# Qualcomm-AI-research/fastforward

Hardware: AMD Instinct MI355X
Metric: tokens/sec Llama-3-8B W8A8 quantized fwd; quant/dequant GB/s vs HBM peak (higher is better)
Workload: dtype int8; 1 GPU; llama3-8b shapes, W8 per-channel symmetric + A8 per-tensor asymmetric on the 7 linears x 32 layers (BASELINE.json configs[2] forward), weights re-quantized every step as in the reference; global_batch=8, seq_len=2048, parallelism=dp1 (batch-sharded replicas, no data-path collective), quantizers=448, launch=hipGraph replay

## Files before the change

fastforward_amd/csrc/ffq_common.h:

```cpp
#pragma once

#include <hip/hip_runtime.h>
#include <stdarg.h>
#include <stdint.h>
#include <stdio.h>

#include "../../include/ffq.h"

#ifndef FFQ_TICKET_ORDER
#define FFQ_TICKET_ORDER __ATOMIC_RELAXED
#endif
#define ffq_ticket_acquire()                                                      \
  do {                                                                            \
    if (FFQ_TICKET_ORDER != __ATOMIC_RELAXED) __builtin_amdgcn_fence(__ATOMIC_ACQUIRE, "agent"); \
  } while (0)

namespace ffq {

char* err_buf();
int fail(int code, const char* fmt, ...);
bool generic_kernels_forced();
bool mid_register_form_forced();
bool splitk_abandon_forced();
int check_launch(const char* what);

__host__ __device__ inline bool dt_valid(int dt) { return dt >= FFQ_F32 && dt <= FFQ_U8; }
__host__ __device__ inline bool dt_is_float(int dt) {
  return dt == FFQ_F32 || dt == FFQ_BF16 || dt == FFQ_F16 || dt == FFQ_F64;
}
__host__ __device__ inline int dt_size(int dt) {
  switch (dt) {
    case FFQ_F32: case FFQ_I32: return 4;
    case FFQ_BF16: case FFQ_F16: case FFQ_I16: return 2;
    case FFQ_F64: case FFQ_I64: return 8;
    default: return 1;
  }
}

__host__ __device__ inline float bf16_bits_to_f32(uint16_t h) {
  return __builtin_bit_cast(float, (uint32_t)h << 16);
}
__host__ __device__ inline uint16_t f32_to_bf16_bits(float f) {
  uint32_t u = __builtin_bit_cast(uint32_t, f);
  if (f != f) return 0x7FC0;
  u += 0x7FFFu + ((u >> 16) & 1u);
  return (uint16_t)(u >> 16);
}
__host__ __device__ inline float f16_bits_to_f32(uint16_t h) {
  return (float)__builtin_bit_cast(_Float16, h);
}
__host__ __device__ inline uint16_t f32_to_f16_bits(float f) {
  return __builtin_bit_cast(uint16_t, (_Float16)f);
}

__host__ __device__ inline float round_stage(float v, int dt) {
  if (dt == FFQ_BF16) return bf16_bits_to_f32(f32_to_bf16_bits(v));
  if (dt == FFQ_F16) return f16_bits_to_f32(f32_to_f16_bits(v));
  return v;
}

__host__ __device__ inline float rne(float v) { return __builtin_rintf(v); }
__host__ __device__ inline double rne(double v) { return __builtin_rint(v); }

__host__ __device__ inline float clamp_nan(float v, float lo, float hi) {
  float c = v < lo ? lo : v;
  c = c > hi ? hi : c;
  return v != v ? v : c;
}
__host__ __device__ inline double clamp_nan(double v, double lo, double hi) {
  double c = v < lo ? lo : v;
  c = c > hi ? hi : c;
  return v != v ? v : c;
}

__device__ inline double load_any(const void* p, int dt, int64_t i) {
  switch (dt) {
    case FFQ_F32: return (double)((const float*)p)[i];
    case FFQ_BF16: return (double)bf16_bits_to_f32(((const uint16_t*)p)[i]);
    case FFQ_F16: return (double)f16_bits_to_f32(((const uint16_t*)p)[i]);
    case FFQ_F64: return ((const double*)p)[i];
    case FFQ_I8: return (double)((const int8_t*)p)[i];
    case FFQ_I16: return (double)((const int16_t*)p)[i];
    case FFQ_I32: return (double)((const int32_t*)p)[i];
    case FFQ_I64: return (double)((const int64_t*)p)[i];
    default: return (double)((const uint8_t*)p)[i];
  }
}
__device__ inline void store_any(void* p, int dt, int64_t i, double v) {
  const bool nan = v != v;
  switch (dt) {
    case FFQ_F32: ((float*)p)[i] = (float)v; break;
    case FFQ_BF16: ((uint16_t*)p)[i] = f32_to_bf16_bits((float)v); break;
    case FFQ_F16: ((uint16_t*)p)[i] = f32_to_f16_bits((float)v); break;
    case FFQ_F64: ((double*)p)[i] = v; break;
    case FFQ_I8: ((int8_t*)p)[i] = nan ? 0 : (int8_t)(int64_t)v; break;
    case FFQ_I16: ((int16_t*)p)[i] = nan ? 0 : (int16_t)(int64_t)v; break;
    case FFQ_I32: ((int32_t*)p)[i] = nan ? INT32_MIN : (int32_t)(int64_t)v; break;
    case FFQ_I64: ((int64_t*)p)[i] = nan ? INT64_MIN : (int64_t)v; break;
    default: ((uint8_t*)p)[i] = nan ? 0 : (uint8_t)(int64_t)v; break;
  }
}

struct FastDiv {
  uint32_t mul;
  uint32_t shift;
  uint32_t div;
// ... 103 lines not shown
```

fastforward_amd/csrc/ffq_core.hip:

```cpp
#include "ffq_common.h"

#include <math.h>
#include <string.h>

namespace ffq {

static thread_local char g_err[512];

char* err_buf() { return g_err; }

int fail(int code, const char* fmt, ...) {
  va_list ap;
  va_start(ap, fmt);
  vsnprintf(g_err, sizeof g_err, fmt, ap);
  va_end(ap);
  return code;
}

int check_launch(const char* what) {
  hipError_t e = hipGetLastError();
  if (e != hipSuccess) return fail(FFQ_ERR_LAUNCH, "%s: %s", what, hipGetErrorString(e));
  return FFQ_OK;
}

// ... 85 lines not shown
                what, (long long)numel);
  return fail(FFQ_ERR_PARAM_NUMEL,
              "The size of tensor a (%lld) must match the size of tensor b (%lld) at non-singleton "
              "dimension 0 (%s vs number of tiles)",
              (long long)ntiles, (long long)numel, what);
}

GenericTiling make_generic(const ffq_tiling* t) {
  GenericTiling g;
  memset(&g, 0, sizeof g);
  g.ndim = t->ndim;
  int64_t s = 1;
  for (int k = t->ndim - 1; k >= 0; --k) {
    g.shape[k] = t->shape[k];
    g.tile[k] = t->tile[k];
    g.gstride[k] = s;
    s *= t->shape[k] / t->tile[k];
  }
  return g;
}

}

using namespace ffq;

extern "C" {

int ffq_abi_version(void) { return FFQ_ABI_VERSION; }
const char* ffq_last_error(void) { return err_buf(); }
const char* ffq_backend_name(void) { return "hip:gfx950"; }

int64_t ffq_num_tiles(const ffq_tiling* tiling) {
  TileInfo info;
  int rc = analyse(tiling, &info);
  if (rc) return -rc;
  return info.ntiles;
}

int ffq_promote_types(int a, int b) {
  if (!dt_valid(a) || !dt_valid(b)) return -FFQ_ERR_ARG;
  if (a == b) return a;
  const bool fa = dt_is_float(a), fb = dt_is_float(b);
  if (fa && !fb) return a;
  if (fb && !fa) return b;
  if (fa && fb) {
    if (a == FFQ_F64 || b == FFQ_F64) return FFQ_F64;
    return FFQ_F32;
  }
  if (a == FFQ_I64 || b == FFQ_I64) return FFQ_I64;
  if (a == FFQ_I32 || b == FFQ_I32) return FFQ_I32;
  return FFQ_I16;
}

int ffq_can_support_bitwidth(int dtype, double num_bits) {
  double avail;
  switch (dtype) {
    case FFQ_BF16: avail = 7; break;
    case FFQ_F16: avail = 10; break;
    case FFQ_F32: avail = 23; break;
    case FFQ_F64: avail = 52; break;
    case FFQ_I8: case FFQ_U8: avail = 8; break;
    case FFQ_I16: avail = 16; break;
    case FFQ_I32: avail = 32; break;
    case FFQ_I64: avail = 64; break;
    default: return 0;
  }
  return (avail + 2) >= num_bits;
}

int ffq_dequantize_result_dtype(int data_dt, int scale_dt, int offset_dt, int has_offset) {
  const int off_dt = has_offset ? offset_dt : scale_dt;
  const int add_dt = ffq_promote_types(data_dt, off_dt);
  if (add_dt < 0) return add_dt;
  return ffq_promote_types(add_dt, scale_dt);
}

}

namespace ffq {
static int g_force_generic = 0;
bool generic_kernels_forced() { return (__atomic_load_n(&g_force_generic, __ATOMIC_RELAXED) & 1) != 0; }
bool splitk_abandon_forced() { return (__atomic_load_n(&g_force_generic, __ATOMIC_RELAXED) & 2) != 0; }
bool mid_register_form_forced() { return (__atomic_load_n(&g_force_generic, __ATOMIC_RELAXED) & 4) != 0; }
}

extern "C" int ffq_force_generic_kernels(int on) {
  return __atomic_exchange_n(&ffq::g_force_generic, on & 7, __ATOMIC_RELAXED);
}
```

fastforward_amd/csrc/ffq_linear.hip:

```cpp
#include "ffq_affine.h"
#include "ffq_common.h"
#include "ffq_vec.h"
#include "ffq_epilogue.h"
#include "ffq_extrema.h"
#include "ffq_silu.h"

#include <math.h>

#include <type_traits>

namespace ffq {

typedef int v4i __attribute__((ext_vector_type(4)));
typedef int v16i __attribute__((ext_vector_type(16)));

constexpr int BM = 128, BN = 128, BK = 64;
constexpr int kTileBytes = BM * BK;
constexpr int64_t kMaxContraction = 131071;

struct LinearArgs {
  const int8_t* xq;
  const int8_t* wq;
  const float* x_scale; const float* x_offset;
  const float* w_scale; const float* w_offset;
// ... 494 lines not shown
  const int r16 = lane & 15, g4 = lane >> 4;
  const int col0 = n0 + wn * 32;
  bf16_t* out = static_cast<bf16_t*>(a.out);
#pragma unroll
  for (int half = 0; half < 2; ++half) {
#pragma unroll
    for (int nj = 0; nj < 2; ++nj) {
      const int cb = 16 * nj + 4 * g4;
      fq_f32x2 CG[2], OG[2], CU[2], OU[2];
#pragma unroll
      for (int t = 0; t < 4; t += 2) {
        const int n = col0 + cb + t;
        CG[t >> 1] = fq_f32x2{sx * a.w_scale[n], sx * a.w_scale[n + 1]};
        CU[t >> 1] = fq_f32x2{sx * a.w_scale2[n], sx * a.w_scale2[n + 1]};
        OG[t >> 1] = fq_f32x2{ox * rs_lds[cb + t], ox * rs_lds[cb + t + 1]};
        OU[t >> 1] = fq_f32x2{ox * rs_lds[32 + cb + t], ox * rs_lds[32 + cb + t + 1]};
      }
      uint32_t wg[4][2], ws[4][2];
      uint32_t bad = 0;
#pragma unroll
      for (int q = 0; q < 4; ++q) {
        const int mi = 4 * half + q;
#pragma unroll
        for (int t = 0; t < 4; t += 2) {
          const fq_f32x2 A = {(float)acc[mi][nj][t], (float)acc[mi][nj][t + 1]};
          const fq_f32x2 G = CG[t >> 1] * (A + OG[t >> 1]);
          wg[q][t >> 1] = pack2<bf16_t>(G.x, G.y);
          ws[q][t >> 1] = silu_pair_lookup(wg[q][t >> 1], silu_table, bad);
        }
      }
      if (__builtin_expect(silu_any_outside(bad), 0)) {
#pragma unroll
        for (int q = 0; q < 4; ++q)
#pragma unroll
          for (int h2 = 0; h2 < 2; ++h2) ws[q][h2] = silu_pair_patch(wg[q][h2], ws[q][h2]);
      }
#pragma unroll
      for (int q = 0; q < 4; ++q) {
        const int mi = 4 * half + q;
        u32x2 zw;
#pragma unroll
        for (int t = 0; t < 4; t += 2) {
          const fq_f32x2 A = {(float)acc[mi][nj + 2][t], (float)acc[mi][nj + 2][t + 1]};
          const fq_f32x2 U = CU[t >> 1] * (A + OU[t >> 1]);
          uint32_t w = pack2<bf16_t>(U.x, U.y);
          const fq_f32x2 UB = {__builtin_bit_cast(float, w << 16), __builtin_bit_cast(float, w & 0xFFFF0000u)};
          w = ws[q][t >> 1];
          const fq_f32x2 SB = {__builtin_bit_cast(float, w << 16), __builtin_bit_cast(float, w & 0xFFFF0000u)};
          const fq_f32x2 Z = SB * UB;
          w = pack2<bf16_t>(Z.x, Z.y);
          if (t == 0) zw.x = w; else zw.y = w;
        }
        const int rowl = wm * 64 + q * 16 + r16;
        *reinterpret_cast<u32x2*>(lds2 + rowl * PITCH + wn * 64 + cb * 2) = zw;
      }
    }
    __syncthreads();
#pragma unroll 1
    for (int t = 0; t < 4; ++t) {
      const int idx = wave * 256 + t * 64 + lane;
      const int rowl = idx >> 4, seg = idx & 15;
      const int m = m0 + (rowl >> 6) * 128 + half * 64 + (rowl & 63);
      const u32x4 v = *reinterpret_cast<const u32x4*>(lds2 + rowl * PITCH + seg * 16);
      if (m < a.M) {
        __builtin_nontemporal_store(v, reinterpret_cast<u32x4*>(reinterpret_cast<uint8_t*>(out) + ((size_t)m * a.N + n0) * 2 + seg * 16));
        if (a.extrema.words) {
          const uint32_t vw[4] = {v.x, v.y, v.z, v.w};
          float zmn = zext[0], zmx = zext[512], znan = zext[1024];
#pragma unroll
          for (int q = 0; q < 4; ++q) {
            const float z0 = __builtin_bit_cast(float, vw[q] << 16), z1 = __builtin_bit_cast(float, vw[q] & 0xFFFF0000u);
            zmn = __builtin_fminf(zmn, __builtin_fminf(z0, z1));
            zmx = __builtin_fmaxf(zmx, __builtin_fmaxf(z0, z1));
            znan = (z0 != z0 || z1 != z1) ? 1.0f : znan;
          }
          zext[0] = zmn; zext[512] = zmx; zext[1024] = znan;
        }
      }
    }
    __syncthreads();
  }
}

template <typename TOut, bool REQUANT, bool MLP, bool WOFF = false, bool GATED = false>
__global__ __launch_bounds__(512, 2) void w8a8_gemm256fq_kernel(LinearArgs a, int total_tiles) {
  constexpr int BN2 = 256, WAVES_N = 4;
  constexpr int BN_OUT = MLP ? 128 : 256;
  constexpr int SLOT_BYTES = (BM2 + BN2) * 128;
  constexpr int B_IMAGE = BM2 * 128;
  extern __shared__ __attribute__((aligned(16))) uint8_t lds2[];

  const int tid = threadIdx.x, lane = tid & 63;
  const int wave = __builtin_amdgcn_readfirstlane(tid >> 6);
  const int wm = wave / WAVES_N, wn = wave % WAVES_N;

  const uint32_t nblk = gridDim.x;
  const uint32_t xcd = blockIdx.x & 7u, j_in_xcd = blockIdx.x >> 3;
  const uint32_t blocks_in_xcd = (nblk >> 3) + (xcd < (nblk & 7u) ? 1u : 0u);
  const uint32_t tq = (uint32_t)total_tiles >> 3, tr = (uint32_t)total_tiles & 7u;
  const uint32_t xcd_first = xcd < tr ? xcd * (tq + 1) : tr * (tq + 1) + (xcd - tr) * tq;
  const uint32_t xcd_count = tq + (xcd < tr ? 1u : 0u);
  const int my_tiles = j_in_xcd < xcd_count ? (int)((xcd_count - j_in_xcd + blocks_in_xcd - 1) / blocks_in_xcd) : 0;
  constexpr bool PRODUCT = MLP && !REQUANT;
  if constexpr (WOFF || GATED || PRODUCT) {
    if (a.run_if && *a.run_if != a.run_when) return;
  }
  const int8_t* xq_in_force = a.xq;
  if constexpr (WOFF || GATED) {
    const uint64_t p = reinterpret_cast<uint64_t>(codes_in_force(a.xq, a.x_scale, a.x_offset, a.earlier));
    const uint32_t lo = __builtin_amdgcn_readfirstlane((uint32_t)p), hi = __builtin_amdgcn_readfirstlane((uint32_t)(p >> 32));
    xq_in_force = reinterpret_cast<const int8_t*>(((uint64_t)hi << 32) | lo);
  }
  if (my_tiles == 0) {
    if constexpr (GATED || PRODUCT) {
      if (a.extrema.words && tid == 0) extrema_publish(a.extrema, 0.0f, 0.0f, false, false, gridDim.x);
    }
    return;
  }
  uint16_t* const silu_table = reinterpret_cast<uint16_t*>(lds2 + 2 * SLOT_BYTES);
  [[maybe_unused]] float* const zext = reinterpret_cast<float*>(lds2 + 2 * SLOT_BYTES + kSiluBytes) + tid;
  if constexpr (GATED || PRODUCT) {
    zext[0] = INFINITY; zext[512] = -INFINITY; zext[1024] = 0.0f;
  }
  if constexpr (MLP || GATED) silu_table_fill(silu_table, (uint32_t)tid, 512u);

  const int k_rot = (!GATED && a.K >= 8192 && (a.K & (a.K - 1)) == 0) ? (int)(xcd * (uint32_t)(a.K / 128) / 8u) : 0;
  const int d_row = lane >> 3;
  uint32_t a_voff[4], b_voff[4];
  const int8_t* a_base = xq_in_force;
  const int8_t* b_base[4];
  int m0 = 0, n0 = 0;
  auto tile_origin = [&](int it, int& tm0, int& tn0) {
    const uint32_t tile_id = xcd_first + j_in_xcd + (uint32_t)it * blocks_in_xcd;
    const uint32_t gm = (uint32_t)a.group_m;
    const uint32_t across = a.group_cols ? (uint32_t)a.tiles_m : (uint32_t)a.tiles_n;
    const uint32_t along = a.group_cols ? (uint32_t)a.tiles_n : (uint32_t)a.tiles_m;
    const uint32_t per_group = gm * across;
    const uint32_t group = tile_id / per_group, in_group = tile_id - group * per_group;
    const uint32_t group_size = min(gm, along - group * gm);
    const uint32_t inner = group * gm + in_group % group_size, outer = in_group / group_size;
    tm0 = (int)(a.group_cols ? outer : inner) * BM2;
    tn0 = (int)(a.group_cols ? inner : outer) * BN_OUT;
  };
  auto row_base = [&](const int8_t* base, int row0) {
    const uint64_t off = (uint64_t)(uint32_t)row0 * (uint64_t)(uint32_t)a.K;
    const uint32_t lo = __builtin_amdgcn_readfirstlane((uint32_t)off), hi = __builtin_amdgcn_readfirstlane((uint32_t)(off >> 32));
    return base + (((uint64_t)hi << 32) | lo);
  };
  auto set_sources = [&](int tm0, int tn0) {
    a_base = row_base(xq_in_force, tm0);
#pragma unroll
    for (int c = 0; c < 4; ++c) {
      const int row = (wave * 4 + c) * 8 + d_row;
      const int d_slot = (lane & 7) ^ ((row >> 1) & 7);
      int ra = row;
      ra = tm0 + ra < a.M ? ra : a.M - 1 - tm0;
      if constexpr (GATED) a_voff[c] = __umul24((uint32_t)ra, (uint32_t)a.K) + (uint32_t)(d_slot * 16);
      else a_voff[c] = (uint32_t)ra * (uint32_t)a.K + d_slot * 16;
      if constexpr (MLP) {
        const int rb = (row >> 6) * 32 + (row & 31);
        b_base[c] = row_base((((wave * 4 + c) * 8) & 32) ? a.wq2 : a.wq, tn0);
        b_voff[c] = (uint32_t)rb * (uint32_t)a.K + d_slot * 16;
      } else {
        int rb = row;
        rb = tn0 + rb < a.N ? rb : a.N - 1 - tn0;
        b_base[c] = row_base(a.wq, tn0);
        if constexpr (GATED) b_voff[c] = __umul24((uint32_t)rb, (uint32_t)a.K) + (uint32_t)(d_slot * 16);
        else b_voff[c] = (uint32_t)rb * (uint32_t)a.K + d_slot * 16;
      }
    }
  };
  auto issue_a = [&](int ks, int slot, int c0) {
    uint8_t* base = lds2 + slot * SLOT_BYTES;
#pragma unroll
    for (int c = c0; c < c0 + 2; ++c) {
      asm volatile("" : "+v"(a_voff[c]));
      __builtin_amdgcn_global_load_lds((gbl_void_t*)((a_base + ks * 128) + a_voff[c]), (lds_void_t*)(base + (wave * 4 + c) * 1024), 16, 0, 0);
    }
  };
  auto issue_b = [&](int ks, int slot, int c0) {
    uint8_t* base = lds2 + slot * SLOT_BYTES + B_IMAGE;
#pragma unroll
    for (int c = c0; c < c0 + 2; ++c) {
      asm volatile("" : "+v"(b_voff[c]));
      __builtin_amdgcn_global_load_lds((gbl_void_t*)((b_base[c] + ks * 128) + b_voff[c]), (lds_void_t*)(base + (wave * 4 + c) * 1024), 16, 0, 0);
    }
  };

  const uint32_t r16 = lane & 15, g4 = lane >> 4;
  uint32_t a_off[2], b_off[2];
  {
    const uint32_t arow = wm * 128 + r16, brow = wn * 64 + r16;
#pragma unroll
    for (int kq = 0; kq < 2; ++kq) {
      a_off[kq] = arow * 128 + (((kq * 4 + g4) ^ ((arow >> 1) & 7u)) << 4);
      b_off[kq] = B_IMAGE + brow * 128 + (((kq * 4 + g4) ^ ((brow >> 1) & 7u)) << 4);
    }
  }

  v4i32 acc[8][4];
  v4i fa[4], fb[4];
  auto read_frags = [&](const uint8_t* st, int phase) {
    const int kq = phase >> 1, mh = phase & 1;
    if (mh == 0) {
#pragma unroll
      for (int nj = 0; nj < 4; ++nj) fb[nj] = *reinterpret_cast<const v4i*>(st + b_off[kq] + nj * 2048);
    }
#pragma unroll
    for (int q = 0; q < 4; ++q) fa[q] = *reinterpret_cast<const v4i*>(st + a_off[kq] + (4 * mh + q) * 2048);
  };
  auto cluster = [&](int mh) {
    asm volatile("s_waitcnt lgkmcnt(0)" ::: "memory");
    __builtin_amdgcn_sched_barrier(0);
    __builtin_amdgcn_s_setprio(1);
#pragma unroll
    for (int q = 0; q < 4; ++q) {
#pragma unroll
      for (int n_ = 0; n_ < 4; ++n_) {
        const int nj = (q & 1) ? 3 - n_ : n_;
        if (mh == 0) acc[q][nj] = __builtin_amdgcn_mfma_i32_16x16x64_i8(fb[nj], fa[q], acc[q][nj], 0, 0, 0);
        else acc[4 + q][nj] = __builtin_amdgcn_mfma_i32_16x16x64_i8(fb[nj], fa[q], acc[4 + q][nj], 0, 0, 0);
      }
    }
    __builtin_amdgcn_sched_barrier(0);
    __builtin_amdgcn_s_setprio(0);
  };

  const int ksuper = a.K / 128;
  int slot = 0;
  tile_origin(0, m0, n0);
  set_sources(m0, n0);
  issue_a(k_rot, 0, 0); issue_a(k_rot, 0, 2); issue_b(k_rot, 0, 0); issue_b(k_rot, 0, 2);
  asm volatile("s_waitcnt vmcnt(0)" ::: "memory");
  __builtin_amdgcn_s_barrier();

  for (int it = 0; it < my_tiles; ++it) {
#pragma unroll
    for (int mi = 0; mi < 8; ++mi)
#pragma unroll
      for (int nj = 0; nj < 4; ++nj)
#pragma unroll
        for (int e = 0; e < 4; ++e) acc[mi][nj][e] = 0;
    int nm0 = m0, nn0 = n0;
    const bool has_next = it + 1 < my_tiles;
    if (has_next) tile_origin(it + 1, nm0, nn0);
    if (wm == 1) __builtin_amdgcn_s_barrier();
    for (int ks = 0; ks < ksuper; ++ks) {
      const uint8_t* st = lds2 + slot * SLOT_BYTES;
      int fetch = ks + 1;
      if (ks == ksuper - 1) {
        fetch = has_next ? 0 : ks;
        if (has_next) set_sources(nm0, nn0);
      }
      fetch += k_rot;
      fetch = fetch >= ksuper ? fetch - ksuper : fetch;
      read_frags(st, 0);
      __builtin_amdgcn_sched_barrier(0);
      asm volatile("s_waitcnt lgkmcnt(0)" ::: "memory");
      issue_a(fetch, slot ^ 1, 0); issue_b(fetch, slot ^ 1, 0);
      __builtin_amdgcn_sched_barrier(0);
      __builtin_amdgcn_s_barrier();
      cluster(0);
      __builtin_amdgcn_s_barrier();
      read_frags(st, 1);
      __builtin_amdgcn_sched_barrier(0);
      asm volatile("s_waitcnt lgkmcnt(0)" ::: "memory");
      issue_a(fetch, slot ^ 1, 2); issue_b(fetch, slot ^ 1, 2);
      __builtin_amdgcn_sched_barrier(0);
      __builtin_amdgcn_s_barrier();
      cluster(1);
      __builtin_amdgcn_s_barrier();
      read_frags(st, 2);
      __builtin_amdgcn_sched_barrier(0);
      __builtin_amdgcn_s_barrier();
      cluster(0);
      __builtin_amdgcn_s_barrier();
      read_frags(st, 3);
      asm volatile("s_waitcnt vmcnt(0)" ::: "memory");
      __builtin_amdgcn_sched_barrier(0);
      __builtin_amdgcn_s_barrier();
      cluster(1);
      __builtin_amdgcn_s_barrier();
      slot ^= 1;
    }
    if (wm == 0) __builtin_amdgcn_s_barrier();
    uint8_t* scratch = lds2 + (slot ^ 1) * SLOT_BYTES;
    __syncthreads();
    if constexpr (MLP) {
      int rsw[2] = {0, 0};
      if (a.rowsum_w) {
        rsw[0] = a.rowsum_w[n0 + wn * 32 + (lane & 31)];
        rsw[1] = a.rowsum_w2[n0 + wn * 32 + (lane & 31)];
      }
#ifdef FFQ_ABLATE_EPILOGUE
      {
        int sum = rsw[0];
#pragma unroll
        for (int mi = 0; mi < 8; ++mi)
#pragma unroll
          for (int nj = 0; nj < 4; ++nj) sum += (acc[mi][nj][0] ^ acc[mi][nj][1]) + (acc[mi][nj][2] ^ acc[mi][nj][3]);
        if (sum == 0x7fffffff) static_cast<int8_t*>(a.out)[lane] = (int8_t)sum;
      }
#else
      if constexpr (REQUANT) mlp_epilogue16_body(a, acc, rsw, scratch, wave, lane, wm, wn, m0, n0, silu_table);
      else mlp_epilogue16_product(a, acc, rsw, scratch, wave, lane, wm, wn, m0, n0, silu_table, zext);
#endif
    } else {
#ifdef FFQ_ABLATE_EPILOGUE
      {
        int sum = 0;
#pragma unroll
        for (int mi = 0; mi < 8; ++mi)
#pragma unroll
          for (int nj = 0; nj < 4; ++nj) sum += (acc[mi][nj][0] ^ acc[mi][nj][1]) + (acc[mi][nj][2] ^ acc[mi][nj][3]);
        if (sum == 0x7fffffff) static_cast<int8_t*>(a.out)[lane] = (int8_t)sum;
      }
#else
      gemm256_epilogue_slabs16<TOut, REQUANT, WOFF, GATED>(a, acc, scratch, wave, lane, wm, wn, m0, n0, silu_table, zext);
#endif
    }
    __syncthreads();
    m0 = nm0; n0 = nn0;
  }
  if constexpr (GATED || PRODUCT) {
    if (a.extrema.words) {
      float mn = zext[0], mx = zext[512], nan = zext[1024];
#pragma unroll
      for (int d = 32; d >= 1; d >>= 1) {
        mn = __builtin_fminf(mn, __shfl_xor(mn, d, 64));
        mx = __builtin_fmaxf(mx, __shfl_xor(mx, d, 64));
        nan = __builtin_fmaxf(nan, __shfl_xor(nan, d, 64));
      }
      float* red = reinterpret_cast<float*>(lds2);
      if (lane == 0) { red[wave] = mn; red[8 + wave] = mx; red[16 + wave] = nan; }
      __syncthreads();
      if (tid == 0) {
        for (int w = 1; w < 8; ++w) {
          mn = __builtin_fminf(mn, red[w]);
          mx = __builtin_fmaxf(mx, red[8 + w]);
          nan = __builtin_fmaxf(nan, red[16 + w]);
        }
        extrema_publish(a.extrema, mn, mx, nan != 0.0f, true, gridDim.x);
      }
    }
  }
}

__global__ __launch_bounds__(256) void rowsum_i8_kernel(const int8_t* __restrict__ q, int rows, int K,
                                                        int32_t* __restrict__ sums, const int32_t* __restrict__ gate,
                                                        const float* __restrict__ offsets = nullptr, int n_offsets = 0,
                                                        int32_t* __restrict__ flag = nullptr, EarlierCodes earlier = {nullptr, nullptr, nullptr},
                                                        const float* __restrict__ q_scale = nullptr, const float* __restrict__ q_offset = nullptr) {
  if (offsets && blockIdx.x == 0) {
    int any = 0;
    for (int i = threadIdx.x; i < n_offsets; i += 256) any |= rne(offsets[i]) != 0.0f;
    any = __syncthreads_or(any);
    if (threadIdx.x == 0) flag[0] = any ? 1 : 0;
  }
  if (gate && *gate == 0) return;
  if (earlier.codes) q = codes_in_force(q, q_scale, q_offset, earlier);
  const int row = blockIdx.x * 4 + (threadIdx.x >> 6);
  const int lane = threadIdx.x & 63;
  int s = 0;
  if (row < rows) {
    const int8_t* p = q + (size_t)row * K;
    for (int k = lane * 16; k < K; k += 64 * 16) {
      const u32x4 v = *reinterpret_cast<const u32x4*>(p + k);
      s = __builtin_amdgcn_sdot4((int)v.x, 0x01010101, s, false);
      s = __builtin_amdgcn_sdot4((int)v.y, 0x01010101, s, false);
      s = __builtin_amdgcn_sdot4((int)v.z, 0x01010101, s, false);
      s = __builtin_amdgcn_sdot4((int)v.w, 0x01010101, s, false);
    }
  }
#pragma unroll
  for (int d = 32; d >= 1; d >>= 1) s += __shfl_xor(s, d, 64);
  if (lane == 0 && row < rows) sums[row] = s;
}

__global__ __launch_bounds__(1024) void offsets_nonzero_kernel(const float* __restrict__ offset, int n, int32_t* __restrict__ flag) {
  int any = 0;
  for (int i = threadIdx.x; i < n; i += 1024) any |= rne(offset[i]) != 0.0f;
  any = __syncthreads_or(any);
  if (threadIdx.x == 0) flag[0] = any ? 1 : 0;
}

}

using namespace ffq;

static int64_t tiles(int64_t extent, int64_t tile) { return (extent + tile - 1) / tile; }

static bool persistent_class(int64_t M, int64_t N, int64_t K) {
  if (M <= 0 || N <= 0 || K <= 0) return false;
  return K % 128 == 0 && K >= 256 && M >= 128 && N >= 128 && tiles(M, BM2) * tiles(N, 256) >= 64;
}

extern "C" int ffq_linear_w8a8_takes_earlier(int64_t M, int64_t N, int64_t K) { return persistent_class(M, N, K) ? 1 : 0; }

static int walk_group_m(int64_t K) { return K >= 8192 ? 4 : GROUP_M2; }

constexpr size_t persistent_lds(bool silu_table, bool extrema) {
  return (size_t)2 * (BM2 + 256) * 128 + (silu_table ? kSiluBytes : 0) + (extrema ? 3 * 512 * 4 : 0);
}

template <typename T, bool RQ, bool MLP, bool WO = false, bool GATED = false>
static void launch_persistent(const LinearArgs& a, hipStream_t s) {
  constexpr size_t lds = persistent_lds(MLP || GATED, GATED || (MLP && !RQ));
  const unsigned total = (unsigned)(a.tiles_m * a.tiles_n);
  static uint64_t attr_set = 0;
  ensure_dynamic_lds(&attr_set, reinterpret_cast<const void*>(&w8a8_gemm256fq_kernel<T, RQ, MLP, WO, GATED>), (int)lds);
  w8a8_gemm256fq_kernel<T, RQ, MLP, WO, GATED><<<total < 256u ? total : 256u, 512, lds, s>>>(a, (int)total);
}

static int launch_tile_kernel(const LinearArgs& a, dim3 grid, hipStream_t s, const char* what);

static LinearArgs linear_args(int64_t M, int64_t N, int64_t K) {
  LinearArgs a{};
  a.M = (int)M; a.N = (int)N; a.K = (int)K;
  a.group_m = GROUP_M2;
  a.seg_start[0] = a.seg_start[1] = INT32_MAX;
  return a;
}

static void set_output(LinearArgs& a, void* out, int out_dt, const float* out_scale, const float* out_offset, double out_num_bits, int y_dt) {
  a.out = out; a.out_dt = out_dt;
  a.out_scale = out_scale; a.out_offset = out_offset;
  const double lo = -pow(2.0, out_num_bits - 1.0);
  a.out_lo = (float)lo; a.out_hi = (float)(-lo - 1.0);
  a.y_dt = y_dt;
}

static int check_extents(int64_t batch, int64_t M, int64_t N, int64_t K, bool* empty) {
  *empty = batch == 0 || M == 0 || N == 0;
  return batch < 0 || M < 0 || N < 0 || K < 0 ? fail(FFQ_ERR_ARG, "negative extent") : FFQ_OK;
}

static int check_contraction(int64_t M, int64_t N, int64_t K) {
  if (M > INT32_MAX || N > INT32_MAX || K > INT32_MAX) return fail(FFQ_ERR_ARG, "extent exceeds 2^31");
  if (K > kMaxContraction) return fail(FFQ_ERR_DTYPE, "K = %lld exceeds %lld (the int32 accumulator's bound: 2^14 * K must stay below 2^31)", (long long)K, (long long)kMaxContraction);
  return FFQ_OK;
}

static int check_codes(const char* what, const char* operands, int64_t K, bool aligned) {
  return K % 16 != 0 || !aligned ? fail(FFQ_ERR_DTYPE, "%s needs K %% 16 == 0 and 16-byte aligned %s", what, operands) : FFQ_OK;
}

static bool real_dt(int dt) { return dt == FFQ_F32 || dt == FFQ_BF16 || dt == FFQ_F16; }

static int check_output(const char* result, int out_dt, bool requant, double out_num_bits, int y_dt) {
  if (!requant) return real_dt(out_dt) ? FFQ_OK : fail(FFQ_ERR_DTYPE, "real-valued output must be f32, bf16 or f16");
  if (!ffq_can_support_bitwidth(out_dt, out_num_bits))
    return fail(FFQ_ERR_PRECISION, "Provided dtype (%d) is not enough to store %g bits quantized values.", out_dt, out_num_bits);
  return real_dt(y_dt) ? FFQ_OK : fail(FFQ_ERR_DTYPE, "the re-quantized %s's real-valued dtype must be f32, bf16 or f16", result);
}

static int check_workspace(bool needed, const char* what, size_t need, const void* workspace, size_t workspace_bytes) {
  return needed && (need > workspace_bytes || !workspace) ? fail(FFQ_ERR_WORKSPACE, "%s needs %zu workspace bytes, got %zu", what, need, workspace_bytes) : FFQ_OK;
}

static size_t round256(int64_t bytes) { return (size_t)((bytes + 255) & ~(int64_t)255); }

struct LinearWorkspace { int32_t* rowsum_x; int32_t* rowsum_w; int32_t* flag; size_t bytes; };
static LinearWorkspace linear_workspace(void* base, int64_t M, int64_t N) {
  int32_t* ws = static_cast<int32_t*>(base);
  return {ws, ws ? ws + M : nullptr, ws ? ws + M + N : nullptr, round256((M + N + 1) * 4)};
}

struct GateUpWorkspace { int32_t* rowsum_gate; int32_t* rowsum_up; size_t bytes; };
static GateUpWorkspace gate_up_workspace(void* base, int64_t N) {
  int32_t* ws = static_cast<int32_t*>(base);
  return {ws, ws ? ws + N : nullptr, round256(2 * N * 4)};
}

struct EstimatingWorkspace { int32_t* flag; GateUpWorkspace sums; void* linear; size_t linear_bytes; size_t bytes; };
static EstimatingWorkspace estimating_workspace(void* base, int64_t M, int64_t N) {
  char* p = static_cast<char*>(base);
  const GateUpWorkspace sums = gate_up_workspace(p ? p + 256 : nullptr, N);
  const size_t linear_bytes = linear_workspace(nullptr, M, N).bytes;
  return {reinterpret_cast<int32_t*>(p), sums, p ? p + 256 + sums.bytes : nullptr, linear_bytes, 256 + sums.bytes + linear_bytes};
}

extern "C" size_t ffq_linear_w8a8_workspace_bytes(int64_t M, int64_t N, int64_t K) {
  (void)K;
  return M < 0 || N < 0 ? 0 : linear_workspace(nullptr, M, N).bytes;
}

struct LinearOptions {
  const void* gate = nullptr;
  uint32_t* extrema_words = nullptr; void* extrema_pair = nullptr;
  const int32_t* run_if = nullptr; int run_when = 0;
  EarlierCodes earlier = {nullptr, nullptr, nullptr};
  int seg_count = 1; const int64_t* seg_ns = nullptr; void* const* seg_outs = nullptr;
};

static int linear_w8a8_impl(const int8_t* xq, const int8_t* wq, const int32_t* w_rowsum, const float* x_scale,
                            const float* x_offset, int x_per_row, const float* w_scale, const float* w_offset,
                            int w_per_row, const void* bias, int bias_dt, void* out, int out_dt,
                            const float* out_scale, const float* out_offset, double out_num_bits, int y_dt, int64_t M,
                            int64_t N, int64_t K, void* workspace, size_t workspace_bytes, void* stream, const LinearOptions& o = {}) {
  hipStream_t s = static_cast<hipStream_t>(stream);
  const bool persistent = persistent_class(M, N, K), requant = out_scale != nullptr;
  bool empty;
  if (int rc = check_extents(1, M, N, K, &empty); rc || empty) return rc;
  if (o.earlier.codes && (!o.earlier.scale || x_per_row || !aligned16(o.earlier.codes) || !persistent))
    return fail(FFQ_ERR_DTYPE, "earlier codes: per-tensor activation parameters on the persistent kernel's shapes (ffq_linear_w8a8_takes_earlier)");
  if (!xq || !wq || !x_scale || !w_scale || !out) return fail(FFQ_ERR_ARG, "NULL buffer");
  if (int rc = check_contraction(M, N, K)) return rc;
  if (int rc = check_codes("w8a8 linear", "code pointers", K, aligned16(xq) && aligned16(wq))) return rc;
  if (bias && !dt_valid(bias_dt)) return fail(FFQ_ERR_ARG, "bad bias dtype");
  if (int rc = check_output("linear", out_dt, requant, out_num_bits, y_dt)) return rc;
  const LinearWorkspace ws = linear_workspace(workspace, M, N);
  if (int rc = check_workspace((x_offset && !w_rowsum && persistent) || w_offset || o.earlier.codes, "w8a8 linear", ws.bytes, workspace, workspace_bytes)) return rc;

  LinearArgs a = linear_args(M, N, K);
  a.xq = xq; a.wq = wq;
  a.x_scale = x_scale; a.x_offset = x_offset; a.x_per_row = x_per_row;
  a.w_scale = w_scale; a.w_offset = w_offset; a.w_per_row = w_per_row;
  a.bias = bias; a.bias_dt = bias_dt;
  set_output(a, out, out_dt, out_scale, out_offset, out_num_bits, y_dt);
  a.gate = static_cast<const bf16_t*>(o.gate);
  a.run_if = o.run_if; a.run_when = o.run_when;
  a.earlier = o.earlier;
  a.extrema = {o.extrema_words, o.extrema_pair, FFQ_BF16};

  if (o.gate && !(persistent && N % 64 == 0 && out_dt == FFQ_BF16 && !requant && !bias && aligned16(o.gate) && aligned16(out)))
    return fail(FFQ_ERR_DTYPE, "gated w8a8 linear: outside the persistent kernel's whole-line path (bf16 out, N %% 64 == 0, >= 64 tiles of 256 x 256)");
  if (o.seg_count > 1) {
    if (!persistent || requant || w_offset || o.gate || o.earlier.codes) return fail(FFQ_ERR_DTYPE, "w8a8 linears in one launch: the persistent kernel's plain form only (>= 64 tiles, no weight offsets, no output quantizer)");
    int64_t at = 0;
    for (int i = 0; i + 1 < o.seg_count; ++i) {
      if (o.seg_ns[i] % 256 != 0) return fail(FFQ_ERR_DTYPE, "w8a8 linears in one launch: every weight matrix but the last needs a multiple of 256 rows");
      at += o.seg_ns[i];
      a.seg_start[i] = (int)at;
      a.seg_out[i] = o.seg_outs[i + 1];
    }
  }
  bool flag_written = false;
  if (x_offset) {
    if (w_rowsum) {
      a.rowsum_w = w_rowsum;
    } else if (!persistent) {
      a.rowsum_w_inside = 1;
    } else {
      flag_written = w_offset != nullptr;
      rowsum_i8_kernel<<<(unsigned)((N + 3) / 4), 256, 0, s>>>(wq, (int)N, (int)K, ws.rowsum_w, nullptr, w_offset, w_per_row ? (int)N : 1,
                                                               flag_written ? ws.flag : nullptr);
      a.rowsum_w = ws.rowsum_w;
    }
  }
  if (w_offset) {
    if (persistent) {
      if (!flag_written) offsets_nonzero_kernel<<<1, 1024, 0, s>>>(w_offset, w_per_row ? (int)N : 1, ws.flag);
      rowsum_i8_kernel<<<(unsigned)((M + 3) / 4), 256, 0, s>>>(xq, (int)M, (int)K, ws.rowsum_x, ws.flag, nullptr, 0, nullptr, o.earlier, x_scale, x_offset);
      a.woff_live = ws.flag;
    } else {
      rowsum_i8_kernel<<<(unsigned)((M + 3) / 4), 256, 0, s>>>(xq, (int)M, (int)K, ws.rowsum_x, nullptr);
    }
    a.rowsum_x = ws.rowsum_x;
  }

  if (!persistent) {
    a.tiles_m = (int)tiles(M, BM);
    a.tiles_n = (int)tiles(N, BN);
    return launch_tile_kernel(a, dim3((unsigned)(a.tiles_m * a.tiles_n)), s, "w8a8_gemm_kernel");
  }
  a.tiles_m = (int)tiles(M, BM2);
  a.tiles_n = (int)tiles(N, 256);
  a.group_m = walk_group_m(K);
#ifdef FFQ_I8_GROUP_COLS
  if ((size_t)M * (size_t)K > ((size_t)200 << 20)) { a.group_cols = 1; a.group_m = FFQ_I8_GROUP_COLS; }
#endif
  if (o.gate) {
    if (w_offset) launch_persistent<bf16_t, false, false, true, true>(a, s); else launch_persistent<bf16_t, false, false, false, true>(a, s);
    return check_launch("w8a8_gemm256fq_kernel (gated)");
  }
  if (o.run_if && !w_offset) a.woff_live = o.run_if + 1;
  if (o.earlier.codes && !w_offset && !o.run_if) {
    hipError_t e = hipMemsetAsync(ws.flag, 0, 4, s);
    if (e != hipSuccess) return fail(FFQ_ERR_LAUNCH, "hipMemsetAsync: %s", hipGetErrorString(e));
    a.woff_live = ws.flag;
  }
#define FFQ_FQ(T, RQ) do { if (w_offset || o.run_if || o.earlier.codes) launch_persistent<T, RQ, false, true>(a, s); else launch_persistent<T, RQ, false, false>(a, s); } while (0)
  if (requant) {
    switch (out_dt) {
      case FFQ_I8: FFQ_FQ(int8_t, true); break;
      case FFQ_BF16: FFQ_FQ(bf16_t, true); break;
      case FFQ_F16: FFQ_FQ(f16_t, true); break;
      case FFQ_F32: FFQ_FQ(float, true); break;
      default: return fail(FFQ_ERR_DTYPE, "re-quantized output container must be i8, bf16, f16 or f32");
    }
  } else {
    switch (out_dt) {
      case FFQ_BF16: FFQ_FQ(bf16_t, false); break;
      case FFQ_F16: FFQ_FQ(f16_t, false); break;
      default: FFQ_FQ(float, false); break;
    }
  }
#undef FFQ_FQ
  return check_launch("w8a8_gemm256fq_kernel");
}

static int launch_tile_kernel(const LinearArgs& a, dim3 grid, hipStream_t s, const char* what) {
  if (a.out_scale) {
    switch (a.out_dt) {
      case FFQ_I8: w8a8_gemm_kernel<int8_t, true><<<grid, 256, 0, s>>>(a); break;
      case FFQ_BF16: w8a8_gemm_kernel<bf16_t, true><<<grid, 256, 0, s>>>(a); break;
      case FFQ_F16: w8a8_gemm_kernel<f16_t, true><<<grid, 256, 0, s>>>(a); break;
      case FFQ_F32: w8a8_gemm_kernel<float, true><<<grid, 256, 0, s>>>(a); break;
      default: return fail(FFQ_ERR_DTYPE, "re-quantized output container must be i8, bf16, f16 or f32");
    }
  } else {
    switch (a.out_dt) {
      case FFQ_BF16: w8a8_gemm_kernel<bf16_t, false><<<grid, 256, 0, s>>>(a); break;
      case FFQ_F16: w8a8_gemm_kernel<f16_t, false><<<grid, 256, 0, s>>>(a); break;
      default: w8a8_gemm_kernel<float, false><<<grid, 256, 0, s>>>(a); break;
    }
  }
  return check_launch(what);
}

extern "C" int ffq_linear_w8a8(const int8_t* xq, const int8_t* wq, const int32_t* w_rowsum, const float* x_scale,
                               const float* x_offset, int x_per_row, const float* w_scale, const float* w_offset,
                               int w_per_row, const void* bias, int bias_dt, void* out, int out_dt,
                               const float* out_scale, const float* out_offset, double out_num_bits, int y_dt, int64_t M,
                               int64_t N, int64_t K, void* workspace, size_t workspace_bytes, void* stream) {
  return linear_w8a8_impl(xq, wq, w_rowsum, x_scale, x_offset, x_per_row, w_scale, w_offset, w_per_row, bias, bias_dt, out, out_dt, out_scale,
                          out_offset, out_num_bits, y_dt, M, N, K, workspace, workspace_bytes, stream);
}

extern "C" int ffq_linear_w8a8_multi(const int8_t* xq, const int8_t* wq, const int32_t* w_rowsum, const float* x_scale, const float* x_offset,
                                     int x_per_row, const float* w_scale, int count, void* const* outs, int out_dt, int64_t M, const int64_t* Ns,
                                     int64_t K, void* workspace, size_t workspace_bytes, void* stream) {
  if (count < 2 || count > 3 || !outs || !Ns) return fail(FFQ_ERR_ARG, "2 or 3 weight matrices");
  int64_t N = 0;
  for (int i = 0; i < count; ++i) {
    if (Ns[i] <= 0 || !outs[i]) return fail(FFQ_ERR_ARG, "empty weight matrix or NULL output");
    if (!aligned16(outs[i])) return fail(FFQ_ERR_DTYPE, "w8a8 linears in one launch need 16-byte aligned outputs");
    N += Ns[i];
  }
  LinearOptions o;
  o.seg_count = count; o.seg_ns = Ns; o.seg_outs = outs;
  return linear_w8a8_impl(xq, wq, w_rowsum, x_scale, x_offset, x_per_row, w_scale, nullptr, 1, nullptr, 0, outs[0], out_dt, nullptr, nullptr, 8.0, 0, M, N, K,
                          workspace, workspace_bytes, stream, o);
}

extern "C" int ffq_linear_w8a8_earlier(const int8_t* xq, const int8_t* earlier_xq, const float* earlier_scale, const float* earlier_offset,
                                       const int8_t* wq, const int32_t* w_rowsum, const float* x_scale, const float* x_offset,
                                       const float* w_scale, const float* w_offset, int w_per_row, void* out, int out_dt, int64_t M,
                                       int64_t N, int64_t K, void* workspace, size_t workspace_bytes, void* stream) {
  if (!earlier_xq || !earlier_scale) return fail(FFQ_ERR_ARG, "NULL earlier codes / scale");
  LinearOptions o;
  o.earlier = {earlier_xq, earlier_scale, earlier_offset};
  return linear_w8a8_impl(xq, wq, w_rowsum, x_scale, x_offset, 0, w_scale, w_offset, w_per_row, nullptr, 0, out, out_dt, nullptr, nullptr, 8.0, 0,
                          M, N, K, workspace, workspace_bytes, stream, o);
}

extern "C" int ffq_linear_w8a8_gated(const int8_t* xq, const int8_t* wq, const int32_t* w_rowsum, const float* x_scale,
                                     const float* x_offset, int x_per_row, const float* w_scale, const float* w_offset,
                                     int w_per_row, const void* gate, void* out, int64_t M, int64_t N, int64_t K,
                                     void* workspace, size_t workspace_bytes, uint32_t* extrema_words, void* extrema_pair, void* stream) {
  if (!gate) return fail(FFQ_ERR_ARG, "NULL gate");
  if ((extrema_words == nullptr) != (extrema_pair == nullptr)) return fail(FFQ_ERR_ARG, "extrema_words and extrema_pair come together");
  LinearOptions o;
  o.gate = gate; o.extrema_words = extrema_words; o.extrema_pair = extrema_pair;
  return linear_w8a8_impl(xq, wq, w_rowsum, x_scale, x_offset, x_per_row, w_scale, w_offset, w_per_row, nullptr, 0, out, FFQ_BF16, nullptr,
// ... 169 lines not shown
```

Measured before the change: 138,100 tokens/s.

## Add three-slot A ring / two-slot B LDS pipeline for large-K persistent W8A8 GEMM

Adds a RING3 variant of the persistent int8 GEMM kernel that splits LDS into three A images and two B images, so A loads are issued two k-steps ahead while B stays double-buffered. It waits on vmcnt(4) instead of draining all loads each step, aiming to hide more global-load latency on large-K plain GEMMs (K>=8192, large operands, e.g. the down projection). The variant uses the full 160KB of LDS, so it can only apply to plain (non-requant, no gate/offset) outputs, and the epilogue reuses the retired ring images as scratch. Debug force flags are added to select or disable the form.

```diff
diff --git a/fastforward_amd/csrc/ffq_common.h b/fastforward_amd/csrc/ffq_common.h
--- a/fastforward_amd/csrc/ffq_common.h
+++ b/fastforward_amd/csrc/ffq_common.h
@@ -22,6 +22,8 @@
 bool generic_kernels_forced();
 bool mid_register_form_forced();
 bool splitk_abandon_forced();
+bool ring3_form_forced();
+bool two_slot_form_forced();
 int check_launch(const char* what);
 
 __host__ __device__ inline bool dt_valid(int dt) { return dt >= FFQ_F32 && dt <= FFQ_U8; }
diff --git a/fastforward_amd/csrc/ffq_core.hip b/fastforward_amd/csrc/ffq_core.hip
--- a/fastforward_amd/csrc/ffq_core.hip
+++ b/fastforward_amd/csrc/ffq_core.hip
@@ -191,8 +191,10 @@
 bool generic_kernels_forced() { return (__atomic_load_n(&g_force_generic, __ATOMIC_RELAXED) & 1) != 0; }
 bool splitk_abandon_forced() { return (__atomic_load_n(&g_force_generic, __ATOMIC_RELAXED) & 2) != 0; }
 bool mid_register_form_forced() { return (__atomic_load_n(&g_force_generic, __ATOMIC_RELAXED) & 4) != 0; }
+bool ring3_form_forced() { return (__atomic_load_n(&g_force_generic, __ATOMIC_RELAXED) & 8) != 0; }
+bool two_slot_form_forced() { return (__atomic_load_n(&g_force_generic, __ATOMIC_RELAXED) & 16) != 0; }
 }
 
 extern "C" int ffq_force_generic_kernels(int on) {
-  return __atomic_exchange_n(&ffq::g_force_generic, on & 7, __ATOMIC_RELAXED);
-}
+  return __atomic_exchange_n(&ffq::g_force_generic, on & 31, __ATOMIC_RELAXED);
+}
diff --git a/fastforward_amd/csrc/ffq_linear.hip b/fastforward_amd/csrc/ffq_linear.hip
--- a/fastforward_amd/csrc/ffq_linear.hip
+++ b/fastforward_amd/csrc/ffq_linear.hip
@@ -600,12 +600,15 @@
   }
 }
 
-template <typename TOut, bool REQUANT, bool MLP, bool WOFF = false, bool GATED = false>
+template <typename TOut, bool REQUANT, bool MLP, bool WOFF = false, bool GATED = false, bool RING3 = false>
 __global__ __launch_bounds__(512, 2) void w8a8_gemm256fq_kernel(LinearArgs a, int total_tiles) {
   constexpr int BN2 = 256, WAVES_N = 4;
   constexpr int BN_OUT = MLP ? 128 : 256;
   constexpr int SLOT_BYTES = (BM2 + BN2) * 128;
   constexpr int B_IMAGE = BM2 * 128;
+  constexpr int IMAGE = BM2 * 128, RING_B0 = 3 * IMAGE;
+  static_assert(!RING3 || (!REQUANT && !MLP && !WOFF && !GATED), "the ring form has no LDS for a table or the extrema");
+  static_assert(BN2 * 128 == IMAGE, "both operands' images are 256 rows of 128 bytes");
   extern __shared__ __attribute__((aligned(16))) uint8_t lds2[];
 
   const int tid = threadIdx.x, lane = tid & 63;
@@ -688,6 +691,42 @@
       }
     }
   };
+  [[maybe_unused]] auto set_sources_a = [&](int tm0) {
+    a_base = row_base(xq_in_force, tm0);
+#pragma unroll
+    for (int c = 0; c < 4; ++c) {
+      const int row = (wave * 4 + c) * 8 + d_row;
+      const int d_slot = (lane & 7) ^ ((row >> 1) & 7);
+      const int ra = tm0 + row < a.M ? row : a.M - 1 - tm0;
+      a_voff[c] = (uint32_t)ra * (uint32_t)a.K + d_slot * 16;
+    }
+  };
+  [[maybe_unused]] auto set_sources_b = [&](int tn0) {
+#pragma unroll
+    for (int c = 0; c < 4; ++c) {
+      const int row = (wave * 4 + c) * 8 + d_row;
+      const int d_slot = (lane & 7) ^ ((row >> 1) & 7);
+      const int rb = tn0 + row < a.N ? row : a.N - 1 - tn0;
+      b_base[c] = row_base(a.wq, tn0);
+      b_voff[c] = (uint32_t)rb * (uint32_t)a.K + d_slot * 16;
+    }
+  };
+  [[maybe_unused]] auto issue_ring_a = [&](int ks, int img, int c0, int n) {
+    uint8_t* base = lds2 + img * IMAGE;
+#pragma unroll
+    for (int c = c0; c < c0 + n; ++c) {
+      asm volatile("" : "+v"(a_voff[c]));
+      __builtin_amdgcn_global_load_lds((gbl_void_t*)((a_base + ks * 128) + a_voff[c]), (lds_void_t*)(base + (wave * 4 + c) * 1024), 16, 0, 0);
+    }
+  };
+  [[maybe_unused]] auto issue_ring_b = [&](int ks, int img, int c0, int n) {
+    uint8_t* base = lds2 + RING_B0 + img * IMAGE;
+#pragma unroll
+    for (int c = c0; c < c0 + n; ++c) {
+      asm volatile("" : "+v"(b_voff[c]));
+      __builtin_amdgcn_global_load_lds((gbl_void_t*)((b_base[c] + ks * 128) + b_voff[c]), (lds_void_t*)(base + (wave * 4 + c) * 1024), 16, 0, 0);
+    }
+  };
   auto issue_a = [&](int ks, int slot, int c0) {
     uint8_t* base = lds2 + slot * SLOT_BYTES;
 #pragma unroll
@@ -712,7 +751,7 @@
 #pragma unroll
     for (int kq = 0; kq < 2; ++kq) {
       a_off[kq] = arow * 128 + (((kq * 4 + g4) ^ ((arow >> 1) & 7u)) << 4);
-      b_off[kq] = B_IMAGE + brow * 128 + (((kq * 4 + g4) ^ ((brow >> 1) & 7u)) << 4);
+      b_off[kq] = (RING3 ? 0 : B_IMAGE) + brow * 128 + (((kq * 4 + g4) ^ ((brow >> 1) & 7u)) << 4);
     }
   }
 
@@ -727,6 +766,15 @@
 #pragma unroll
     for (int q = 0; q < 4; ++q) fa[q] = *reinterpret_cast<const v4i*>(st + a_off[kq] + (4 * mh + q) * 2048);
   };
+  [[maybe_unused]] auto read_frags_ring = [&](const uint8_t* sa, const uint8_t* sb, int phase) {
+    const int kq = phase >> 1, mh = phase & 1;
+    if (mh == 0) {
+#pragma unroll
+      for (int nj = 0; nj < 4; ++nj) fb[nj] = *reinterpret_cast<const v4i*>(sb + b_off[kq] + nj * 2048);
+    }
+#pragma unroll
+    for (int q = 0; q < 4; ++q) fa[q] = *reinterpret_cast<const v4i*>(sa + a_off[kq] + (4 * mh + q) * 2048);
+  };
   auto cluster = [&](int mh) {
     asm volatile("s_waitcnt lgkmcnt(0)" ::: "memory");
     __builtin_amdgcn_sched_barrier(0);
@@ -748,7 +796,13 @@
   int slot = 0;
   tile_origin(0, m0, n0);
   set_sources(m0, n0);
-  issue_a(k_rot, 0, 0); issue_a(k_rot, 0, 2); issue_b(k_rot, 0, 0); issue_b(k_rot, 0, 2);
+  [[maybe_unused]] int ai = 0, bi = 0;
+  if constexpr (RING3) {
+    const int k1 = k_rot + 1 >= ksuper ? k_rot + 1 - ksuper : k_rot + 1;
+    issue_ring_a(k_rot, 0, 0, 4); issue_ring_b(k_rot, 0, 0, 4); issue_ring_a(k1, 1, 0, 4);
+  } else {
+    issue_a(k_rot, 0, 0); issue_a(k_rot, 0, 2); issue_b(k_rot, 0, 0); issue_b(k_rot, 0, 2);
+  }
   asm volatile("s_waitcnt vmcnt(0)" ::: "memory");
   __builtin_amdgcn_s_barrier();
 
@@ -763,46 +817,109 @@
     const bool has_next = it + 1 < my_tiles;
     if (has_next) tile_origin(it + 1, nm0, nn0);
     if (wm == 1) __builtin_amdgcn_s_barrier();
-    for (int ks = 0; ks < ksuper; ++ks) {
-      const uint8_t* st = lds2 + slot * SLOT_BYTES;
-      int fetch = ks + 1;
-      if (ks == ksuper - 1) {
-        fetch = has_next ? 0 : ks;
-        if (has_next) set_sources(nm0, nn0);
-      }
-      fetch += k_rot;
-      fetch = fetch >= ksuper ? fetch - ksuper : fetch;
-      read_frags(st, 0);
-      __builtin_amdgcn_sched_barrier(0);
-      asm volatile("s_waitcnt lgkmcnt(0)" ::: "memory");
-      issue_a(fetch, slot ^ 1, 0); issue_b(fetch, slot ^ 1, 0);
-      __builtin_amdgcn_sched_barrier(0);
-      __builtin_amdgcn_s_barrier();
-      cluster(0);
-      __builtin_amdgcn_s_barrier();
-      read_frags(st, 1);
-      __builtin_amdgcn_sched_barrier(0);
-      asm volatile("s_waitcnt lgkmcnt(0)" ::: "memory");
-      issue_a(fetch, slot ^ 1, 2); issue_b(fetch, slot ^ 1, 2);
-      __builtin_amdgcn_sched_barrier(0);
-      __builtin_amdgcn_s_barrier();
-      cluster(1);
-      __builtin_amdgcn_s_barrier();
-      read_frags(st, 2);
-      __builtin_amdgcn_sched_barrier(0);
-      __builtin_amdgcn_s_barrier();
-      cluster(0);
-      __builtin_amdgcn_s_barrier();
-      read_frags(st, 3);
-      asm volatile("s_waitcnt vmcnt(0)" ::: "memory");
-      __builtin_amdgcn_sched_barrier(0);
-      __builtin_amdgcn_s_barrier();
-      cluster(1);
-      __builtin_amdgcn_s_barrier();
-      slot ^= 1;
+    if constexpr (RING3) {
+      for (int ks = 0; ks < ksuper; ++ks) {
+        const uint8_t* sa = lds2 + ai * IMAGE;
+        const uint8_t* sb = lds2 + RING_B0 + bi * IMAGE;
+        const int a2 = ai == 0 ? 2 : ai - 1;
+        int fetch_b = ks + 1;
+        if (ks == ksuper - 1) {
+          fetch_b = has_next ? 0 : ks;
+          if (has_next) set_sources_b(nn0);
+        }
+        fetch_b += k_rot;
+        fetch_b = fetch_b >= ksuper ? fetch_b - ksuper : fetch_b;
+        int fetch_a = ks + 2;
+        if (fetch_a >= ksuper) {
+          fetch_a = has_next ? fetch_a - ksuper : ks;
+          if (has_next && ks == ksuper - 2) set_sources_a(nm0);
+        }
+        fetch_a += k_rot;
+        fetch_a = fetch_a >= ksuper ? fetch_a - ksuper : fetch_a;
+        read_frags_ring(sa, sb, 0);
+        __builtin_amdgcn_sched_barrier(0);
+        asm volatile("s_waitcnt lgkmcnt(0)" ::: "memory");
+        issue_ring_b(fetch_b, bi ^ 1, 0, 2);
+        __builtin_amdgcn_sched_barrier(0);
+        __builtin_amdgcn_s_barrier();
+        cluster(0);
+        __builtin_amdgcn_s_barrier();
+        read_frags_ring(sa, sb, 1);
+        __builtin_amdgcn_sched_barrier(0);
+        asm volatile("s_waitcnt lgkmcnt(0)" ::: "memory");
+        issue_ring_b(fetch_b, bi ^ 1, 2, 2);
+        __builtin_amdgcn_sched_barrier(0);
+        __builtin_amdgcn_s_barrier();
+        cluster(1);
+        __builtin_amdgcn_s_barrier();
+        read_frags_ring(sa, sb, 2);
+        __builtin_amdgcn_sched_barrier(0);
+        asm volatile("s_waitcnt lgkmcnt(0)" ::: "memory");
+        issue_ring_a(fetch_a, a2, 0, 2);
+        __builtin_amdgcn_sched_barrier(0);
+        __builtin_amdgcn_s_barrier();
+        cluster(0);
+        __builtin_amdgcn_s_barrier();
+        read_frags_ring(sa, sb, 3);
+        __builtin_amdgcn_sched_barrier(0);
+        asm volatile("s_waitcnt lgkmcnt(0)" ::: "memory");
+        issue_ring_a(fetch_a, a2, 2, 2);
+        asm volatile("s_waitcnt vmcnt(4)" ::: "memory");
+        __builtin_amdgcn_sched_barrier(0);
+        __builtin_amdgcn_s_barrier();
+        cluster(1);
+        __builtin_amdgcn_s_barrier();
+        ai = ai == 2 ? 0 : ai + 1;
+        bi ^= 1;
+      }
+    } else {
+      for (int ks = 0; ks < ksuper; ++ks) {
+        const uint8_t* st = lds2 + slot * SLOT_BYTES;
+        int fetch = ks + 1;
+        if (ks == ksuper - 1) {
+          fetch = has_next ? 0 : ks;
+          if (has_next) set_sources(nm0, nn0);
+        }
+        fetch += k_rot;
+        fetch = fetch >= ksuper ? fetch - ksuper : fetch;
+        read_frags(st, 0);
+        __builtin_amdgcn_sched_barrier(0);
+        asm volatile("s_waitcnt lgkmcnt(0)" ::: "memory");
+        issue_a(fetch, slot ^ 1, 0); issue_b(fetch, slot ^ 1, 0);
+        __builtin_amdgcn_sched_barrier(0);
+        __builtin_amdgcn_s_barrier();
+        cluster(0);
+        __builtin_amdgcn_s_barrier();
+        read_frags(st, 1);
+        __builtin_amdgcn_sched_barrier(0);
+        asm volatile("s_waitcnt lgkmcnt(0)" ::: "memory");
+        issue_a(fetch, slot ^ 1, 2); issue_b(fetch, slot ^ 1, 2);
+        __builtin_amdgcn_sched_barrier(0);
+        __builtin_amdgcn_s_barrier();
+        cluster(1);
+        __builtin_amdgcn_s_barrier();
+        read_frags(st, 2);
+        __builtin_amdgcn_sched_barrier(0);
+        __builtin_amdgcn_s_barrier();
+        cluster(0);
+        __builtin_amdgcn_s_barrier();
+        read_frags(st, 3);
+        asm volatile("s_waitcnt vmcnt(0)" ::: "memory");
+        __builtin_amdgcn_sched_barrier(0);
+        __builtin_amdgcn_s_barrier();
+        cluster(1);
+        __builtin_amdgcn_s_barrier();
+        slot ^= 1;
+      }
     }
     if (wm == 0) __builtin_amdgcn_s_barrier();
     uint8_t* scratch = lds2 + (slot ^ 1) * SLOT_BYTES;
+    [[maybe_unused]] int scratch_wave = wave;
+    if constexpr (RING3) {
+      const int last_a = ai == 0 ? 2 : ai - 1, last_b = bi ^ 1;
+      scratch = wave < 4 ? lds2 + last_a * IMAGE : lds2 + RING_B0 + last_b * IMAGE;
+      scratch_wave = wave & 3;
+    }
     __syncthreads();
     if constexpr (MLP) {
       int rsw[2] = {0, 0};
@@ -834,7 +951,7 @@
         if (sum == 0x7fffffff) static_cast<int8_t*>(a.out)[lane] = (int8_t)sum;
       }
 #else
-      gemm256_epilogue_slabs16<TOut, REQUANT, WOFF, GATED>(a, acc, scratch, wave, lane, wm, wn, m0, n0, silu_table, zext);
+      gemm256_epilogue_slabs16<TOut, REQUANT, WOFF, GATED>(a, acc, scratch, RING3 ? scratch_wave : wave, lane, wm, wn, m0, n0, silu_table, zext);
 #endif
     }
     __syncthreads();
@@ -913,21 +1030,45 @@
   return K % 128 == 0 && K >= 256 && M >= 128 && N >= 128 && tiles(M, BM2) * tiles(N, 256) >= 64;
 }
 
+static bool persistent_kernel_can_run(int64_t M, int64_t N, int64_t K) { return K % 128 == 0 && K >= 256 && M >= 128 && N >= 128; }
+
 extern "C" int ffq_linear_w8a8_takes_earlier(int64_t M, int64_t N, int64_t K) { return persistent_class(M, N, K) ? 1 : 0; }
 
 static int walk_group_m(int64_t K) { return K >= 8192 ? 4 : GROUP_M2; }
 
-constexpr size_t persistent_lds(bool silu_table, bool extrema) {
-  return (size_t)2 * (BM2 + 256) * 128 + (silu_table ? kSiluBytes : 0) + (extrema ? 3 * 512 * 4 : 0);
-}
-
-template <typename T, bool RQ, bool MLP, bool WO = false, bool GATED = false>
+#ifndef FFQ_RING3_MIN_K
+#define FFQ_RING3_MIN_K 8192
+#endif
+#ifndef FFQ_RING3_MIN_BYTES
+#define FFQ_RING3_MIN_BYTES ((int64_t)256 << 20)
+#endif
+static bool ring3_form(int64_t M, int64_t N, int64_t K, bool plain, int segments) {
+  if (!plain) return false;
+  if (two_slot_form_forced()) return false;
+  if (ring3_form_forced()) return true;
+  return segments == 1 && K >= FFQ_RING3_MIN_K && (M + N) * K > FFQ_RING3_MIN_BYTES;
+}
+
+constexpr size_t persistent_lds(bool silu_table, bool extrema, bool ring3 = false) {
+  return (ring3 ? (size_t)5 * BM2 * 128 : (size_t)2 * (BM2 + 256) * 128) + (silu_table ? kSiluBytes : 0) + (extrema ? 3 * 512 * 4 : 0);
+}
+static_assert(persistent_lds(false, false, true) == 160 * 1024, "the ring form takes exactly the CU's LDS");
+
+template <typename T, bool RQ, bool MLP, bool WO = false, bool GATED = false, bool RING3 = false>
 static void launch_persistent(const LinearArgs& a, hipStream_t s) {
-  constexpr size_t lds = persistent_lds(MLP || GATED, GATED || (MLP && !RQ));
+  constexpr size_t lds = persistent_lds(MLP || GATED, GATED || (MLP && !RQ), RING3);
   const unsigned total = (unsigned)(a.tiles_m * a.tiles_n);
   static uint64_t attr_set = 0;
-  ensure_dynamic_lds(&attr_set, reinterpret_cast<const void*>(&w8a8_gemm256fq_kernel<T, RQ, MLP, WO, GATED>), (int)lds);
-  w8a8_gemm256fq_kernel<T, RQ, MLP, WO, GATED><<<total < 256u ? total : 256u, 512, lds, s>>>(a, (int)total);
+  ensure_dynamic_lds(&attr_set, reinterpret_cast<const void*>(&w8a8_gemm256fq_kernel<T, RQ, MLP, WO, GATED, RING3>), (int)lds);
+  w8a8_gemm256fq_kernel<T, RQ, MLP, WO, GATED, RING3><<<total < 256u ? total : 256u, 512, lds, s>>>(a, (int)total);
+}
+
+template <typename T, bool RQ>
+static void launch_persistent_plain(const LinearArgs& a, hipStream_t s, bool ring3) {
+  if constexpr (!RQ) {
+    if (ring3) return launch_persistent<T, false, false, false, false, true>(a, s);
+  }
+  launch_persistent<T, RQ, false, false>(a, s);
 }
 
 static int launch_tile_kernel(const LinearArgs& a, dim3 grid, hipStream_t s, const char* what);
@@ -1017,7 +1158,10 @@
                             const float* out_scale, const float* out_offset, double out_num_bits, int y_dt, int64_t M,
                             int64_t N, int64_t K, void* workspace, size_t workspace_bytes, void* stream, const LinearOptions& o = {}) {
   hipStream_t s = static_cast<hipStream_t>(stream);
-  const bool persistent = persistent_class(M, N, K), requant = out_scale != nullptr;
+  const bool requant = out_scale != nullptr;
+  const bool plain = !requant && !w_offset && !o.gate && !o.run_if && !o.earlier.codes;
+  const bool persistent = persistent_class(M, N, K) ||
+                          (plain && (ring3_form_forced() || two_slot_form_forced()) && persistent_kernel_can_run(M, N, K) && (!x_offset || w_rowsum));
   bool empty;
   if (int rc = check_extents(1, M, N, K, &empty); rc || empty) return rc;
   if (o.earlier.codes && (!o.earlier.scale || x_per_row || !aligned16(o.earlier.codes) || !persistent))
@@ -1088,6 +1232,10 @@
 #ifdef FFQ_I8_GROUP_COLS
   if ((size_t)M * (size_t)K > ((size_t)200 << 20)) { a.group_cols = 1; a.group_m = FFQ_I8_GROUP_COLS; }
 #endif
+  const bool ring3 = ring3_form(M, N, K, plain, o.seg_count);
+#ifdef FFQ_RING3_GROUP_M
+  if (ring3) a.group_m = FFQ_RING3_GROUP_M;
+#endif
   if (o.gate) {
     if (w_offset) launch_persistent<bf16_t, false, false, true, true>(a, s); else launch_persistent<bf16_t, false, false, false, true>(a, s);
     return check_launch("w8a8_gemm256fq_kernel (gated)");
@@ -1098,7 +1246,7 @@
     if (e != hipSuccess) return fail(FFQ_ERR_LAUNCH, "hipMemsetAsync: %s", hipGetErrorString(e));
     a.woff_live = ws.flag;
   }
-#define FFQ_FQ(T, RQ) do { if (w_offset || o.run_if || o.earlier.codes) launch_persistent<T, RQ, false, true>(a, s); else launch_persistent<T, RQ, false, false>(a, s); } while (0)
+#define FFQ_FQ(T, RQ) do { if (w_offset || o.run_if || o.earlier.codes) launch_persistent<T, RQ, false, true>(a, s); else launch_persistent_plain<T, RQ>(a, s, ring3); } while (0)
   if (requant) {
     switch (out_dt) {
       case FFQ_I8: FFQ_FQ(int8_t, true); break;
```

Result: faster. 140,600 tokens/s, median of 6 (+1.8%).
